# umutdundar99/progressive-stable-diffusion

Measured on AMD Instinct MI355X. Metric: images/sec at 512x512, 50 DDIM steps, bs/GPU=4, higher is better.
Workload: dtype f16; 1 GPU; 512x512, 50 DDIM steps, bs=4/GPU, delta-steer lambda=3.0, routing gates on, conditioning prep + VAE decode included; global_batch=4, parallelism=batch-shard x1 + 1 all-gather of uint8 frames

## Files before the change

### progressive-stable-diffusion_amd/csrc/conv_halo.hip

```cpp
#include <cstdlib>
#include <type_traits>

#include "dadd_common.h"
#include "igemm_args.h"
#include "igemm_epilogue.h"

#ifndef DADD_IGEMM_EXP
#define DADD_IGEMM_EXP 0
#endif
#if DADD_IGEMM_EXP == 3
#define DADD_STAMP(var) const unsigned long long var = __builtin_amdgcn_s_memtime()
#define DADD_ACC(dst, a, b) dst += (b) - (a)
#else
#define DADD_STAMP(var)
#define DADD_ACC(dst, a, b)
#endif

namespace {

constexpr int BM = 128, BK = 64, BN = 160;
constexpr int WN = BN / 2, J = WN / 16, NBJ = BN / 32;
constexpr int B_BYTES = BN * BK * 2;
constexpr int W_RING = 4 * B_BYTES;
constexpr int HALO_MAX_PIX = 272;
// ... 250 lines not shown
        __builtin_amdgcn_sched_barrier(0);
      }
      ++gi;
      __builtin_amdgcn_sched_barrier(0);
    };
    for (int c = c0; c < c1; ++c) {
      tap2(std::integral_constant<int, 0>{});
      tap2(std::integral_constant<int, 1>{});
      tap2(std::integral_constant<int, 2>{});
      tap2(std::integral_constant<int, 3>{});
      tap2(std::integral_constant<int, 4>{});
      tap2(std::integral_constant<int, 5>{});
      tap2(std::integral_constant<int, 6>{});
      tap2(std::integral_constant<int, 7>{});
      tap2(std::integral_constant<int, 8>{});
      const char* sw = hb;
      hb = hbo;
      hbo = sw;
    }
    __builtin_amdgcn_s_barrier();
    f4* park = reinterpret_cast<f4*>(smem + wave * (J * 4 * 64 * 16));
    if (wave_all >= 4) {
#pragma unroll
      for (int j = 0; j < J; ++j)
#pragma unroll
        for (int i = 0; i < 4; ++i) park[(j * 4 + i) * 64 + lane] = acc[j][i];
    }
    __builtin_amdgcn_s_barrier();
    if (wave_all >= 4) return;
#pragma unroll
    for (int j = 0; j < J; ++j)
#pragma unroll
      for (int i = 0; i < 4; ++i) acc[j][i] += park[(j * 4 + i) * 64 + lane];
    igemm_epilogue<J, 4, 64, WN>(p, acc, m0, n0, wm, wn, lane, z, smem, nullptr, nullptr, smem + GN_OFF);
    return;
  }
  if constexpr (GNIN) {
    const int cg = Cin >> 5;
    const int g = wave * 8 + (lane >> 3), sub = lane & 7;
    const bool second = p.C2 > 0 && g * cg >= p.C1;
    const float* wsp = second ? p.gni_ws2 : p.gni_ws;
    const int nch = second ? p.gni_nchunk2 : p.gni_nchunk;
    const int wsrc = (second ? p.C2 : p.C1) >> 5;
    const int r = p.C2 > 0 ? cg / wsrc : 1;
    const int g0 = p.C2 > 0 ? ((second ? g * cg - p.C1 : g * cg) / wsrc) : g;
    double a = 0.0, q = 0.0;
    for (int j = 0; j < r; ++j)
      for (int k = sub; k < nch; k += 32) {
        dadd_f2 v[4];
#pragma unroll
        for (int u = 0; u < 4; ++u) {
          const int kk = min(k + 8 * u, nch - 1);
          v[u] = *reinterpret_cast<const dadd_f2*>(wsp + (((size_t)b * nch + kk) * 32 + g0 + j) * 2);
        }
#pragma unroll
        for (int u = 0; u < 4; ++u) {
          if (k + 8 * u < nch) {
            a += (double)v[u][0];
            q += (double)v[u][1];
          }
        }
      }
#pragma unroll
    for (int o = 4; o > 0; o >>= 1) {
      a += __shfl_xor(a, o, 64);
      q += __shfl_xor(q, o, 64);
    }
// ... 112 lines not shown
```

### progressive-stable-diffusion_amd/csrc/igemm.hip

```cpp
#include "dadd_common.h"
#include "igemm_args.h"
#include <cstdlib>
#include <string>
#include "igemm_epilogue.h"

namespace {

constexpr int BM = 128;
constexpr int BK = 64;

__device__ __forceinline__ int lds_off(int row, int chunk) {
  return (row * 8 + (chunk ^ ((row >> 1) & 7))) * 8;
}

template <int BM, int BN, bool DEEP>
__global__ __launch_bounds__(256, 2) void igemm_kernel(const IgemmArgs p) {
  constexpr int WM = BM / 2;
  constexpr int MI = WM / 16;
  constexpr int WN = BN / 2;
  constexpr int J = WN / 16;
  constexpr int NA = BM * 8 / 256;
  constexpr int NB = BN * 8 / 256;
  extern __shared__ __attribute__((aligned(16))) char smem[];
  half_t* As = reinterpret_cast<half_t*>(smem);
  half_t* Bs = As + 2 * BM * BK;

  const int t = threadIdx.x, lane = t & 63, wave = t >> 6;
  const int wm = wave >> 1, wn = wave & 1;
  const int tile_id = xcd_remap(blockIdx.x, gridDim.x);
  int nt, mt;
  tile_decode_fast(p, tile_id, mt, nt);
  const int m0 = mt * BM, n0 = nt * BN;
  const int z = blockIdx.y;
  const int kt0 = z * p.kps;
  const int kt1 = min(p.nkt, kt0 + p.kps);
  const int Cin = p.C1 + p.C2;
  const int q = t & 7;
  const int r0 = t >> 3;
  const int Hv = p.ups ? 2 * p.Hi : p.Hi;
  const int Wv = p.ups ? 2 * p.Wi : p.Wi;
  const int HoWo = p.Ho * p.Wo;

  int a_pix[NA], a_y[NA], a_x[NA];
#pragma unroll
  for (int i = 0; i < NA; ++i) {
    const int m = m0 + r0 + 32 * i;
    const bool ok = m < p.M;
    const int mm = ok ? m : 0;
    int b, oy, ox;
    row_decode(p, mm, HoWo, b, oy, ox);
    a_pix[i] = b * p.Hi * p.Wi;
    a_y[i] = ok ? oy * p.stride - p.pad : -100000;
    a_x[i] = ox * p.stride - p.pad;
// ... 83 lines not shown
      const bool more = kt + 1 < kt1;
      if (more) gload(kt + 1, ra, rb);
      compute(cur);
      if (more) lstore(cur ^ 1, ra, rb);
      __syncthreads();
    }
  } else {
    h8 raA[NA], rbA[NB], raB[NA], rbB[NB];
    if (kt0 < kt1) {
      gload(kt0, raA, rbA);
      if (kt0 + 1 < kt1) gload(kt0 + 1, raB, rbB);
      lstore(0, raA, rbA);
    }
    __syncthreads();
    int kt = kt0;
    while (kt < kt1) {
      if (kt + 2 < kt1) gload(kt + 2, raA, rbA);
      compute(0);
      if (kt + 1 < kt1) lstore(1, raB, rbB);
      __syncthreads();
      if (++kt >= kt1) break;
      if (kt + 2 < kt1) gload(kt + 2, raB, rbB);
      compute(1);
      if (kt + 1 < kt1) lstore(0, raA, rbA);
      __syncthreads();
      ++kt;
    }
  }

  if (ln_stage) {
    asm volatile("s_waitcnt vmcnt(0)" ::: "memory");
    __syncthreads();
  }
  igemm_epilogue<J, MI, WM, WN>(p, acc, m0, n0, wm, wn, lane, z, smem, nullptr, nullptr, ln_scr, ln_sts ? ln_scr + LN_LDS_STATS : nullptr,
                                ln_stage ? ln_scr : nullptr);
}

__global__ __launch_bounds__(256) void splitk_finish_kernel(const IgemmArgs p, int nsplit) {
  const int n4 = p.N >> 2;
  const size_t total = (size_t)p.M * n4;
  const int HoWo = p.Ho * p.Wo;
  for (size_t idx = (size_t)blockIdx.x * blockDim.x + threadIdx.x; idx < total;
       idx += (size_t)gridDim.x * blockDim.x) {
    const int m = (int)(idx / n4);
    const int n = (int)(idx - (size_t)m * n4) * 4;
    f4 v = {0.f, 0.f, 0.f, 0.f};
    const float* slab = p.partial + (size_t)m * p.N + n;
    const size_t sstride = (size_t)p.M * p.N;
    int s = 0;
    for (; s + 4 <= nsplit; s += 4) {
      const f4 t0 = *reinterpret_cast<const f4*>(slab + (size_t)s * sstride);
      const f4 t1 = *reinterpret_cast<const f4*>(slab + (size_t)(s + 1) * sstride);
      const f4 t2 = *reinterpret_cast<const f4*>(slab + (size_t)(s + 2) * sstride);
      const f4 t3 = *reinterpret_cast<const f4*>(slab + (size_t)(s + 3) * sstride);
      v += t0;
      v += t1;
      v += t2;
      v += t3;
    }
    for (; s < nsplit; ++s) v += *reinterpret_cast<const f4*>(slab + (size_t)s * sstride);
    if (p.flags & DADD_EPI_BIAS) v += *reinterpret_cast<const f4*>(p.bias + n);
    if (p.flags & DADD_EPI_ROWVEC)
      v += *reinterpret_cast<const f4*>(p.rowvec + (size_t)(m / HoWo) * p.ld_rowvec + n);
    if (p.flags & DADD_EPI_RESIDUAL) {
      const h4 rv = *reinterpret_cast<const h4*>(p.residual + (size_t)m * p.ldr + n);
#pragma unroll
      for (int r = 0; r < 4; ++r) v[r] += (float)rv[r];
// ... 483 lines not shown
```

### progressive-stable-diffusion_amd/csrc/igemm_dma.hip

```cpp
#include "dadd_common.h"
#include "igemm_args.h"
#include <cstdlib>
#include "igemm_epilogue.h"

namespace {

constexpr int BK = 64;

typedef __attribute__((address_space(3))) void* lptr_t;
constexpr unsigned OOB = 0x80000000u;

__device__ __forceinline__ int lds_off(int row, int chunk) {
  return (row * 8 + (chunk ^ ((row >> 1) & 7))) * 8;
}

template <int N>
__device__ __forceinline__ void wait_vmcnt() {
  asm volatile("s_waitcnt vmcnt(%0)" ::"n"(N) : "memory");
}

template <int BM, int BN, bool UPS, bool PERS, int LNK>
__global__ __launch_bounds__(512, (BM + BN) <= 128 ? 4 : 2) void igemm_dma_kernel(const IgemmArgs p) {
#if defined(__HIP_DEVICE_COMPILE__)
  constexpr bool WS = true;
  constexpr bool LNF = LNK == 1;
  constexpr int WM = BM / 2, MI = WM / 16;
  constexpr int WN = BN / 2;
  constexpr int J = WN / 16;
  constexpr int NA = BM / 32;
  constexpr int NBJ = BN / 32;
  constexpr int LPT = NA + NBJ;
  constexpr int A_BYTES = BM * BK * 2, B_BYTES = BN * BK * 2, STAGE = A_BYTES + B_BYTES;
  extern __shared__ __attribute__((aligned(1024))) char smem[];

  const int t = threadIdx.x, lane = t & 63;
  const int wave_all = __builtin_amdgcn_readfirstlane(t >> 6);
  const bool loader = WS && wave_all >= 4;
  const int wave = WS ? (wave_all & 3) : wave_all;
  const int wm = wave >> 1, wn = wave & 1;
  int tile_first, tile_count;
  if constexpr (PERS) {
    const int total = p.mtiles * p.ntiles, nwg = gridDim.x;
    const int l = xcd_remap(blockIdx.x, nwg);
    const int q = total / nwg, r = total - q * nwg;
    tile_first = l * q + min(l, r);
    tile_count = q + (l < r ? 1 : 0);
  } else {
    tile_first = xcd_remap(blockIdx.x, gridDim.x);
    tile_count = 1;
  }
  const int z = PERS ? 0 : blockIdx.y;
  const int kt0 = PERS ? 0 : z * p.kps;
  const int kt1 = PERS ? p.nkt : min(p.nkt, kt0 + p.kps);
  const int nk = kt1 - kt0;
  const int Cin = p.C1 + p.C2;
  const int Hv = UPS ? 2 * p.Hi : p.Hi;
  const int Wv = UPS ? 2 * p.Wi : p.Wi;
  const int HoWo = p.Ho * p.Wo;
  const int lrow = lane >> 3, lch = lane & 7;

  const int shift1 = UPS ? 0 : (p.pad * p.Wi + p.pad) * p.C1;
// ... 249 lines not shown
        acc[jj][ii] = DADD_MFMA_16X16X32(wb0[jj], xa0[ii], acc[jj][ii], 0, 0, 0);
        if constexpr (LNF) {
#pragma unroll
          for (int t2 = 0; t2 < LPER; ++t2)
            if (k * LPER + t2 < LQ) ln_acc_pair(xa0[(k * LPER + t2) / 4], (k * LPER + t2) % 4, ls1[(k * LPER + t2) / 4], ls2[(k * LPER + t2) / 4]);
        }
        if (k == 0) wb1[0] = *reinterpret_cast<const h8*>(cb1);
        else if (k <= MI) xa1[k - 1] = *reinterpret_cast<const h8*>(ca + (k - 1) * 2048);
        else if (k < MI + J) wb1[k - MI] = *reinterpret_cast<const h8*>(cb1 + (k - MI) * 2048);
        __builtin_amdgcn_sched_barrier(0);
      }
#pragma unroll
      for (int k = 0; k < MI * J; ++k) {
        const int jj = k / MI, ii = k % MI;
        acc[jj][ii] = DADD_MFMA_16X16X32(wb1[jj], xa1[ii], acc[jj][ii], 0, 0, 0);
        if constexpr (LNF) {
#pragma unroll
          for (int t2 = 0; t2 < LPER; ++t2)
            if (k * LPER + t2 < LQ) ln_acc_pair(xa1[(k * LPER + t2) / 4], (k * LPER + t2) % 4, ls1[(k * LPER + t2) / 4], ls2[(k * LPER + t2) / 4]);
        }
        if (k == 0) wb0[0] = *reinterpret_cast<const h8*>(nb);
        else if (k <= MI) xa0[k - 1] = *reinterpret_cast<const h8*>(na + (k - 1) * 2048);
        else if (k < MI + J) wb0[k - MI] = *reinterpret_cast<const h8*>(nb + (k - MI) * 2048);
        __builtin_amdgcn_sched_barrier(0);
      }
      comp_off = next_off;
      __builtin_amdgcn_sched_barrier(0);
    }
    dadd_pf_drain(pf_sink);
    int nt, mt;
    tile_decode_fast(p, tile_first + tl, mt, nt);
    if constexpr (LNF) {
      ln_finish<MI>(ls1, ls2, p.K, p.ln_eps);
      igemm_epilogue<J, MI, WM, WN>(p, acc, mt * BM, nt * BN, wm, wn, lane, z, smem, ls1, ls2);
    } else {
      igemm_epilogue<J, MI, WM, WN>(p, acc, mt * BM, nt * BN, wm, wn, lane, z, smem, nullptr, nullptr, smem + 4 * STAGE,
                                    ln_sts ? ln_scr + LN_LDS_STATS : nullptr, ln_stage ? ln_scr : nullptr);
    }
  }
#endif
}

constexpr int smem_bytes(int bm, int bn) {
  return 4 * (bm + bn) * BK * 2 + (bm == 128 ? LN_LDS_BYTES : 4096);
}

#define DMA_ROW(BM, BN, UPS, PERS, LNK)                                                                                \
  {DADD_KNAME("igemm_dma_kernel") "<" #BM ", " #BN ", " #UPS ", " #PERS ", " #LNK ">", igemm_dma_kernel<BM, BN, UPS, PERS, LNK>, \
   512, smem_bytes(BM, BN), {BM, BN, UPS, PERS, LNK}}
#define DMA_ROWS2(BM, BN, PERS) DMA_ROW(BM, BN, false, PERS, 0), DMA_ROW(BM, BN, false, PERS, 1)
#define DMA_ROWS3(BM, BN, PERS) DMA_ROWS2(BM, BN, PERS), DMA_ROW(BM, BN, false, PERS, 2)
const IgemmKernel DMA_KERNELS[] = {
    DMA_ROWS3(128, 128, true),  DMA_ROWS3(128, 160, true),
    DMA_ROWS3(128, 128, false), DMA_ROWS3(128, 160, false),
    DMA_ROW(128, 128, true, false, 0), DMA_ROW(128, 160, true, false, 0),
    DMA_ROWS2(64, 64, false), DMA_ROWS2(64, 128, false), DMA_ROWS2(64, 160, false),
};
#undef DMA_ROWS3
#undef DMA_ROWS2
#undef DMA_ROW

}

int dadd_init_igemm_dma() { return dadd_set_max_lds(DMA_KERNELS); }

const IgemmKernel* dadd_igemm_dma_row(int tile_m, int tile_n, bool ups, bool persistent, int lnk) {
  return dadd_find_row(DMA_KERNELS, tile_m, tile_n, ups, persistent, lnk);
}
```

### progressive-stable-diffusion_amd/csrc/igemm_epilogue.h

```cpp
#pragma once
#include "igemm_args.h"
#include "ln_lds.h"

__device__ __forceinline__ float dadd_row16_sum(float v) {
  v += __builtin_bit_cast(float, __builtin_amdgcn_update_dpp(0, __builtin_bit_cast(int, v), 0xB1, 0xF, 0xF, true));
  v += __builtin_bit_cast(float, __builtin_amdgcn_update_dpp(0, __builtin_bit_cast(int, v), 0x4E, 0xF, 0xF, true));
  v += __builtin_bit_cast(float, __builtin_amdgcn_update_dpp(0, __builtin_bit_cast(int, v), 0x141, 0xF, 0xF, true));
  v += __builtin_bit_cast(float, __builtin_amdgcn_update_dpp(0, __builtin_bit_cast(int, v), 0x140, 0xF, 0xF, true));
  return v;
}

template <int J, int MI, int WM, int WN>
__device__ __forceinline__ void igemm_epilogue(const IgemmArgs& p, f4 (&acc)[J][MI], int m0, int n0,
                                               int wm, int wn, int lane, int z, char* smem,
                                               const float* ln_mu = nullptr, const float* ln_rs = nullptr,
                                               char* gn_scratch = nullptr, const char* ln_lds = nullptr,
                                               const char* ln_cb = nullptr) {
  const int g = lane >> 4, mc = lane & 15;
  const int HoWo = p.Ho * p.Wo;
  if (p.splitk > 1) {
#pragma unroll
    for (int i = 0; i < MI; ++i) {
      const int m = m0 + wm * WM + i * 16 + mc;
      if (m >= p.M) continue;
#pragma unroll
      for (int j = 0; j < J; ++j) {
        const int n = n0 + wn * WN + j * 16 + g * 4;
        if (n < p.N) *reinterpret_cast<f4*>(p.partial + ((size_t)z * p.M + m) * p.N + n) = acc[j][i];
      }
    }
    if (p.counters == nullptr) return;
    asm volatile("s_waitcnt vmcnt(0)" ::: "memory");
    __syncthreads();
    volatile int* flag = reinterpret_cast<volatile int*>(smem);
    if (threadIdx.x == 0) {
      __builtin_amdgcn_fence(__ATOMIC_RELEASE, "agent");
      asm volatile("s_waitcnt vmcnt(0)" ::: "memory");
      int* ticket = p.counters + blockIdx.x;
      const int prev = __hip_atomic_fetch_add(ticket, 1, __ATOMIC_RELAXED, __HIP_MEMORY_SCOPE_AGENT);
      const int last = (prev == p.splitk - 1) ? 1 : 0;
      if (last) {
        __builtin_amdgcn_fence(__ATOMIC_ACQUIRE, "agent");
        asm volatile("s_waitcnt vmcnt(0)" ::: "memory");
        __hip_atomic_store(ticket, 0, __ATOMIC_RELAXED, __HIP_MEMORY_SCOPE_AGENT);
      }
      *flag = last;
    }
    __syncthreads();
    if (*flag == 0) return;
#pragma unroll
    for (int i = 0; i < MI; ++i) {
      const int m = m0 + wm * WM + i * 16 + mc;
#pragma unroll
      for (int j = 0; j < J; ++j) {
        const int n = n0 + wn * WN + j * 16 + g * 4;
        f4 v = {0.f, 0.f, 0.f, 0.f};
        if (m < p.M && n < p.N)
          for (int s = 0; s < p.splitk; ++s)
            v += *reinterpret_cast<const f4*>(p.partial + ((size_t)s * p.M + m) * p.N + n);
        acc[j][i] = v;
      }
    }
  }
  if (p.flags & DADD_EPI_GNSTAT) {
    float* scratch = reinterpret_cast<float*>(gn_scratch) + (wm * 2 + wn) * 256;
    const int mrow0 = m0 + wm * WM;
    const int bsmp = row_sample(p, mrow0, HoWo);
#pragma unroll
    for (int j = 0; j < J; ++j) {
      const int n = n0 + wn * WN + j * 16 + g * 4;
      f4 bias4 = {0.f, 0.f, 0.f, 0.f};
      if (p.flags & DADD_EPI_BIAS) bias4 = *reinterpret_cast<const f4*>(p.bias + n);
      if (p.flags & DADD_EPI_ROWVEC) bias4 += *reinterpret_cast<const f4*>(p.rowvec + (size_t)bsmp * p.ld_rowvec + n);
      float cs[4] = {0.f, 0.f, 0.f, 0.f}, cq[4] = {0.f, 0.f, 0.f, 0.f};
#pragma unroll
      for (int i = 0; i < MI; ++i) {
        const int m = mrow0 + i * 16 + mc;
        f4 v = acc[j][i] + bias4;
        if (p.flags & DADD_EPI_RESIDUAL) {
          const h4 rv = *reinterpret_cast<const h4*>(p.residual + (size_t)m * p.ldr + n);
#pragma unroll
          for (int r = 0; r < 4; ++r) v[r] += (float)rv[r];
        }
        h4 o;
#pragma unroll
        for (int r = 0; r < 4; ++r) {
          o[r] = (half_t)v[r];
          const float f = (float)o[r];
          cs[r] += f;
          cq[r] = fmaf(f, f, cq[r]);
        }
        *reinterpret_cast<h4*>(p.out + (size_t)m * p.ldo + n) = o;
      }
#pragma unroll
      for (int r = 0; r < 4; ++r) {
        cs[r] = dadd_row16_sum(cs[r]);
        cq[r] = dadd_row16_sum(cq[r]);
      }
      if (mc == 0) {
#pragma unroll
        for (int r = 0; r < 4; ++r) {
          scratch[(j * 16 + g * 4 + r) * 2] = cs[r];
          scratch[(j * 16 + g * 4 + r) * 2 + 1] = cq[r];
        }
      }
    }
    __builtin_amdgcn_fence(__ATOMIC_RELEASE, "wavefront");
    __builtin_amdgcn_wave_barrier();
    __builtin_amdgcn_fence(__ATOMIC_ACQUIRE, "wavefront");
    const int ngrp = WN / p.gn_cg;
    if (lane < ngrp) {
      float a = 0.f, q = 0.f;
      for (int c = 0; c < p.gn_cg; ++c) {
        a += scratch[(lane * p.gn_cg + c) * 2];
        q += scratch[(lane * p.gn_cg + c) * 2 + 1];
      }
// ... 24 lines not shown
      mrow[i] = min(m0 + wm * WM + i * 16 + mc, p.M - 1);
    }
    if (ln_lds != nullptr) {
      for (int pp = 0; pp < p.ln_parts_in; ++pp)
#pragma unroll
        for (int i = 0; i < MI; ++i) {
          const dadd_f2 v = *reinterpret_cast<const dadd_f2*>(ln_lds + pp * 1024 + (wm * WM + i * 16 + mc) * 8);
          sa[i] += v[0];
          sq[i] += v[1];
        }
    } else
    for (int pp = 0; pp < p.ln_parts_in; pp += 4) {
      dadd_f2 v[4][MI];
#pragma unroll
      for (int u = 0; u < 4; ++u)
#pragma unroll
        for (int i = 0; i < MI; ++i)
          v[u][i] = st[(size_t)min(pp + u, p.ln_parts_in - 1) * p.M + mrow[i]];
#pragma unroll
      for (int u = 0; u < 4; ++u) {
        const float keep = (pp + u < p.ln_parts_in) ? 1.f : 0.f;
#pragma unroll
        for (int i = 0; i < MI; ++i) {
          sa[i] = fmaf(keep, v[u][i][0], sa[i]);
          sq[i] = fmaf(keep, v[u][i][1], sq[i]);
        }
      }
    }
    const float inv = __builtin_amdgcn_rcpf((float)p.K);
#pragma unroll
    for (int i = 0; i < MI; ++i) {
      const float mu = sa[i] * inv;
      lmu[i] = mu;
      lrs[i] = rsqrtf(fmaxf(sq[i] * inv - mu * mu, 0.f) + p.ln_eps);
    }
    fold = true;
  } else {
#pragma unroll
    for (int i = 0; i < MI; ++i) lmu[i] = 0.f, lrs[i] = 1.f;
  }
  if (fold && ln_cb != nullptr) {
#pragma unroll
    for (int i = 0; i < MI; ++i) {
      const int m = m0 + wm * WM + i * 16 + mc;
      if (m >= p.M) continue;
      if (p.flags & DADD_EPI_GEGLU) {
        if constexpr (J == 4) {
#pragma unroll
          for (int j = 0; j < 2; ++j) {
            const int ch = wn * WN + j * 16 + g * 4, cg2 = ch + 32;
            if (n0 + cg2 >= p.N) continue;
            f4 hv = lrs[i] * (acc[j][i] - lmu[i] * *reinterpret_cast<const f4*>(ln_cb + ch * 4));
            f4 gv = lrs[i] * (acc[j + 2][i] - lmu[i] * *reinterpret_cast<const f4*>(ln_cb + cg2 * 4));
            if (p.flags & DADD_EPI_BIAS) {
              hv += *reinterpret_cast<const f4*>(ln_cb + 1024 + ch * 4);
              gv += *reinterpret_cast<const f4*>(ln_cb + 1024 + cg2 * 4);
            }
            const int no = (n0 >> 1) + wn * 32 + j * 16 + g * 4;
            const dadd_f2 g01 = dadd_gelu2(dadd_f2{gv[0], gv[1]}), g23 = dadd_gelu2(dadd_f2{gv[2], gv[3]});
            const h4 o = {(half_t)(hv[0] * g01[0]), (half_t)(hv[1] * g01[1]), (half_t)(hv[2] * g23[0]),
                          (half_t)(hv[3] * g23[1])};
            *reinterpret_cast<h4*>(p.out + (size_t)m * p.ldo + no) = o;
          }
        }
        continue;
      }
#pragma unroll
      for (int j = 0; j < J; ++j) {
        const int c = wn * WN + j * 16 + g * 4, n = n0 + c;
        if (n >= p.N) continue;
        f4 v = lrs[i] * (acc[j][i] - lmu[i] * *reinterpret_cast<const f4*>(ln_cb + c * 4));
        if (p.flags & DADD_EPI_BIAS) v += *reinterpret_cast<const f4*>(ln_cb + 1024 + c * 4);
        if (p.flags & DADD_EPI_ROWVEC) v += *reinterpret_cast<const f4*>(p.rowvec + (size_t)row_sample(p, m, HoWo) * p.ld_rowvec + n);
        if (p.flags & DADD_EPI_ACT_MASK) {
          if (p.flags & DADD_EPI_QUICKGELU) {
#pragma unroll
            for (int r = 0; r < 4; ++r) v[r] = v[r] / (1.0f + __expf(-1.702f * v[r]));
          } else if (p.flags & DADD_EPI_GELU) {
#pragma unroll
            for (int r = 0; r < 4; ++r) v[r] = dadd_gelu(v[r]);
          } else {
#pragma unroll
            for (int r = 0; r < 4; ++r) v[r] = 1.0f / (1.0f + __expf(-v[r]));
          }
        }
        if (p.flags & DADD_EPI_RESIDUAL) {
          const h4 rv = *reinterpret_cast<const h4*>(p.residual + (size_t)m * p.ldr + n);
#pragma unroll
          for (int r = 0; r < 4; ++r) v[r] += (float)rv[r];
        }
        const h4 o = {(half_t)v[0], (half_t)v[1], (half_t)v[2], (half_t)v[3]};
        *reinterpret_cast<h4*>(p.out + (size_t)m * p.ldo + n) = o;
      }
    }
    return;
  }
  if (fold) {
    if (p.flags & DADD_EPI_GEGLU) {
      if constexpr (J == 4) {
#pragma unroll
        for (int j = 0; j < 2; ++j) {
          const int nh = n0 + wn * WN + j * 16 + g * 4;
          const int ng = nh + 32;
          if (ng >= p.N) continue;
          const f4 c1h = *reinterpret_cast<const f4*>(p.ln_c1 + nh), c1g = *reinterpret_cast<const f4*>(p.ln_c1 + ng);
          f4 bh = {0.f, 0.f, 0.f, 0.f}, bg = {0.f, 0.f, 0.f, 0.f};
          if (p.flags & DADD_EPI_BIAS) {
            bh = *reinterpret_cast<const f4*>(p.bias + nh);
            bg = *reinterpret_cast<const f4*>(p.bias + ng);
          }
          const int no = (n0 >> 1) + wn * 32 + j * 16 + g * 4;
#pragma unroll
          for (int i = 0; i < MI; ++i) {
            const int m = m0 + wm * WM + i * 16 + mc;
            if (m >= p.M) continue;
            const f4 hv = lrs[i] * (acc[j][i] - lmu[i] * c1h) + bh;
            const f4 gv = lrs[i] * (acc[j + 2][i] - lmu[i] * c1g) + bg;
            const dadd_f2 g01 = dadd_gelu2(dadd_f2{gv[0], gv[1]}), g23 = dadd_gelu2(dadd_f2{gv[2], gv[3]});
            const h4 o = {(half_t)(hv[0] * g01[0]), (half_t)(hv[1] * g01[1]), (half_t)(hv[2] * g23[0]),
                          (half_t)(hv[3] * g23[1])};
            *reinterpret_cast<h4*>(p.out + (size_t)m * p.ldo + no) = o;
          }
        }
      }
      return;
    }
#pragma unroll
    for (int j = 0; j < J; ++j) {
      const int n = n0 + wn * WN + j * 16 + g * 4;
      if (n >= p.N) continue;
      const f4 c4 = *reinterpret_cast<const f4*>(p.ln_c1 + n);
      f4 b4 = {0.f, 0.f, 0.f, 0.f};
      if (p.flags & DADD_EPI_BIAS) b4 = *reinterpret_cast<const f4*>(p.bias + n);
#pragma unroll
      for (int i = 0; i < MI; ++i) {
        const int m = m0 + wm * WM + i * 16 + mc;
        if (m >= p.M) continue;
        f4 v = lrs[i] * (acc[j][i] - lmu[i] * c4) + b4;
        if (p.flags & DADD_EPI_ROWVEC) v += *reinterpret_cast<const f4*>(p.rowvec + (size_t)row_sample(p, m, HoWo) * p.ld_rowvec + n);
        if (p.flags & DADD_EPI_ACT_MASK) {
          if (p.flags & DADD_EPI_QUICKGELU) {
#pragma unroll
            for (int r = 0; r < 4; ++r) v[r] = v[r] / (1.0f + __expf(-1.702f * v[r]));
          } else if (p.flags & DADD_EPI_GELU) {
#pragma unroll
            for (int r = 0; r < 4; ++r) v[r] = dadd_gelu(v[r]);
          } else {
#pragma unroll
            for (int r = 0; r < 4; ++r) v[r] = 1.0f / (1.0f + __expf(-v[r]));
          }
        }
        if (p.flags & DADD_EPI_RESIDUAL) {
          const h4 rv = *reinterpret_cast<const h4*>(p.residual + (size_t)m * p.ldr + n);
#pragma unroll
          for (int r = 0; r < 4; ++r) v[r] += (float)rv[r];
        }
        const h4 o = {(half_t)v[0], (half_t)v[1], (half_t)v[2], (half_t)v[3]};
        *reinterpret_cast<h4*>(p.out + (size_t)m * p.ldo + n) = o;
      }
    }
    return;
  }
  const bool lnstat = (p.flags & DADD_EPI_LNSTAT) != 0 && n0 + wn * WN < p.N;
#pragma unroll
  for (int i = 0; i < MI; ++i) {
    const int m = m0 + wm * WM + i * 16 + mc;
    if (m >= p.M) continue;
    const int b = (p.flags & DADD_EPI_ROWVEC) ? row_sample(p, m, HoWo) : 0;
    float rs1 = 0.f, rs2 = 0.f;
    if (p.flags & DADD_EPI_GEGLU) {
      if constexpr (J == 4) {
#pragma unroll
        for (int j = 0; j < 2; ++j) {
          const int nh = n0 + wn * WN + j * 16 + g * 4;
          const int ng = nh + 32;
          if (ng >= p.N) continue;
          f4 hv = acc[j][i], gv = acc[j + 2][i];
          if (p.flags & DADD_EPI_BIAS) {
            hv += *reinterpret_cast<const f4*>(p.bias + nh);
            gv += *reinterpret_cast<const f4*>(p.bias + ng);
          }
          const int no = (n0 >> 1) + wn * 32 + j * 16 + g * 4;
          const dadd_f2 g01 = dadd_gelu2(dadd_f2{gv[0], gv[1]}), g23 = dadd_gelu2(dadd_f2{gv[2], gv[3]});
          const h4 o = {(half_t)(hv[0] * g01[0]), (half_t)(hv[1] * g01[1]), (half_t)(hv[2] * g23[0]),
                        (half_t)(hv[3] * g23[1])};
          *reinterpret_cast<h4*>(p.out + (size_t)m * p.ldo + no) = o;
        }
      }
      continue;
    }
#pragma unroll
    for (int j = 0; j < J; ++j) {
      const int n = n0 + wn * WN + j * 16 + g * 4;
      if (n >= p.N) continue;
      f4 v = acc[j][i];
      if (p.flags & DADD_EPI_BIAS) v += *reinterpret_cast<const f4*>(p.bias + n);
      if (p.flags & DADD_EPI_ROWVEC) v += *reinterpret_cast<const f4*>(p.rowvec + (size_t)b * p.ld_rowvec + n);
      if (p.flags & DADD_EPI_ACT_MASK) {
        if (p.flags & DADD_EPI_QUICKGELU) {
#pragma unroll
          for (int r = 0; r < 4; ++r) v[r] = v[r] / (1.0f + __expf(-1.702f * v[r]));
        } else if (p.flags & DADD_EPI_GELU) {
#pragma unroll
          for (int r = 0; r < 4; ++r) v[r] = dadd_gelu(v[r]);
        } else {
#pragma unroll
          for (int r = 0; r < 4; ++r) v[r] = 1.0f / (1.0f + __expf(-v[r]));
        }
      }
      if (p.flags & DADD_EPI_RESIDUAL) {
        const h4 rv = *reinterpret_cast<const h4*>(p.residual + (size_t)m * p.ldr + n);
#pragma unroll
        for (int r = 0; r < 4; ++r) v[r] += (float)rv[r];
      }
      h4 o;
#pragma unroll
      for (int r = 0; r < 4; ++r) {
        o[r] = (half_t)v[r];
        const float f = (float)o[r];
        rs1 += f;
        rs2 = fmaf(f, f, rs2);
      }
      *reinterpret_cast<h4*>(p.out + (size_t)m * p.ldo + n) = o;
    }
    if (lnstat) {
      rs1 = dadd_sum_x16x32(rs1);
      rs2 = dadd_sum_x16x32(rs2);
      if (g == 0) {
        const int part = (n0 + wn * WN) / WN;
        reinterpret_cast<dadd_f2*>(p.ln_stats_out)[(size_t)part * p.M + m] = dadd_f2{rs1, rs2};
      }
    }
  }
}
```

Before: 11.34 images/sec.

## Restructure GEMM epilogue to batch operand loads by tile, row or column

Rewrites the shared GEMM/conv epilogue so bias, rowvec, LN-fold constants and residual loads are hoisted into register arrays. They are issued in batches: the whole tile up front, per row, or per column, with the mode picked at compile time for each kernel variant. Indices are clamped so loads need no guards, and additions use selects. The aim is more memory-level parallelism and less latency exposed in the store-heavy epilogue. The cost is higher register pressure, which could lower occupancy, plus some slight changes to rounding and FMA contraction.

```diff
diff --git a/progressive-stable-diffusion_amd/csrc/conv_halo.hip b/progressive-stable-diffusion_amd/csrc/conv_halo.hip
--- a/progressive-stable-diffusion_amd/csrc/conv_halo.hip
+++ b/progressive-stable-diffusion_amd/csrc/conv_halo.hip
@@ -306,7 +306,7 @@
     for (int j = 0; j < J; ++j)
 #pragma unroll
       for (int i = 0; i < 4; ++i) acc[j][i] += park[(j * 4 + i) * 64 + lane];
-    igemm_epilogue<J, 4, 64, WN>(p, acc, m0, n0, wm, wn, lane, z, smem, nullptr, nullptr, smem + GN_OFF);
+    igemm_epilogue<J, 4, 64, WN, EPI_COLS>(p, acc, m0, n0, wm, wn, lane, z, smem, nullptr, nullptr, smem + GN_OFF);
     return;
   }
   if constexpr (GNIN) {
diff --git a/progressive-stable-diffusion_amd/csrc/igemm.hip b/progressive-stable-diffusion_amd/csrc/igemm.hip
--- a/progressive-stable-diffusion_amd/csrc/igemm.hip
+++ b/progressive-stable-diffusion_amd/csrc/igemm.hip
@@ -19,6 +19,7 @@
   constexpr int MI = WM / 16;
   constexpr int WN = BN / 2;
   constexpr int J = WN / 16;
+  constexpr int EPI = (DEEP && BN == 128) ? EPI_COLS : EPI_TILE;
   constexpr int NA = BM * 8 / 256;
   constexpr int NB = BN * 8 / 256;
   extern __shared__ __attribute__((aligned(16))) char smem[];
@@ -168,7 +169,8 @@
     asm volatile("s_waitcnt vmcnt(0)" ::: "memory");
     __syncthreads();
   }
-  igemm_epilogue<J, MI, WM, WN>(p, acc, m0, n0, wm, wn, lane, z, smem, nullptr, nullptr, ln_scr, ln_sts ? ln_scr + LN_LDS_STATS : nullptr,
+  const int lane_e = __builtin_amdgcn_mbcnt_hi(~0u, __builtin_amdgcn_mbcnt_lo(~0u, 0u));
+  igemm_epilogue<J, MI, WM, WN, EPI>(p, acc, m0, n0, wm, wn, lane_e, z, smem, nullptr, nullptr, ln_scr, ln_sts ? ln_scr + LN_LDS_STATS : nullptr,
                                 ln_stage ? ln_scr : nullptr);
 }
 
diff --git a/progressive-stable-diffusion_amd/csrc/igemm_dma.hip b/progressive-stable-diffusion_amd/csrc/igemm_dma.hip
--- a/progressive-stable-diffusion_amd/csrc/igemm_dma.hip
+++ b/progressive-stable-diffusion_amd/csrc/igemm_dma.hip
@@ -27,6 +27,7 @@
   constexpr int WM = BM / 2, MI = WM / 16;
   constexpr int WN = BN / 2;
   constexpr int J = WN / 16;
+  constexpr int EPI = !PERS ? EPI_TILE : (BN == 160 && LNK == 2) ? EPI_COLS : EPI_ROWS;
   constexpr int NA = BM / 32;
   constexpr int NBJ = BN / 32;
   constexpr int LPT = NA + NBJ;
@@ -342,9 +343,9 @@
     tile_decode_fast(p, tile_first + tl, mt, nt);
     if constexpr (LNF) {
       ln_finish<MI>(ls1, ls2, p.K, p.ln_eps);
-      igemm_epilogue<J, MI, WM, WN>(p, acc, mt * BM, nt * BN, wm, wn, lane, z, smem, ls1, ls2);
+      igemm_epilogue<J, MI, WM, WN, EPI>(p, acc, mt * BM, nt * BN, wm, wn, lane, z, smem, ls1, ls2);
     } else {
-      igemm_epilogue<J, MI, WM, WN>(p, acc, mt * BM, nt * BN, wm, wn, lane, z, smem, nullptr, nullptr, smem + 4 * STAGE,
+      igemm_epilogue<J, MI, WM, WN, EPI>(p, acc, mt * BM, nt * BN, wm, wn, lane, z, smem, nullptr, nullptr, smem + 4 * STAGE,
                                     ln_sts ? ln_scr + LN_LDS_STATS : nullptr, ln_stage ? ln_scr : nullptr);
     }
   }
diff --git a/progressive-stable-diffusion_amd/csrc/igemm_epilogue.h b/progressive-stable-diffusion_amd/csrc/igemm_epilogue.h
--- a/progressive-stable-diffusion_amd/csrc/igemm_epilogue.h
+++ b/progressive-stable-diffusion_amd/csrc/igemm_epilogue.h
@@ -1,6 +1,153 @@
 #pragma once
 #include "igemm_args.h"
 #include "ln_lds.h"
+#include <type_traits>
+
+__device__ __forceinline__ f4 epi_add_if(bool on, const f4& v, const f4& b) {
+#pragma clang fp contract(off)
+  const f4 s = v + b;
+  return on ? s : v;
+}
+__device__ __forceinline__ f4 epi_add_if(bool on, const f4& v, const h4& b) {
+#pragma clang fp contract(off)
+  const f4 s = {v[0] + (float)b[0], v[1] + (float)b[1], v[2] + (float)b[2], v[3] + (float)b[3]};
+  return on ? s : v;
+}
+__device__ __forceinline__ void epi_activate(int flags, f4& v) {
+  if (flags & DADD_EPI_QUICKGELU) {
+#pragma unroll
+    for (int r = 0; r < 4; ++r) v[r] = v[r] / (1.0f + __expf(-1.702f * v[r]));
+  } else if (flags & DADD_EPI_GELU) {
+#pragma unroll
+    for (int r = 0; r < 4; ++r) v[r] = dadd_gelu(v[r]);
+  } else {
+#pragma unroll
+    for (int r = 0; r < 4; ++r) v[r] = 1.0f / (1.0f + __expf(-v[r]));
+  }
+}
+
+constexpr bool epi_ln_var_fused(int J, int MI, int i) { return MI == 2 || (J == 4 && i >= 2); }
+__device__ __forceinline__ float epi_ln_var(bool fused, float ex2, float mu) {
+#pragma clang fp contract(off)
+  const float mu2 = mu * mu;
+  return fused ? fmaf(-mu, mu, ex2) : ex2 - mu2;
+}
+
+enum { EPI_TILE = 0, EPI_ROWS = 1, EPI_COLS = 2 };
+
+template <int J, int MI, int MODE>
+struct EpiOperands {
+  int mcl[MI], ncl[J];
+  f4 b4[J], c4[J], r4[J];
+  f4 rq[MI];
+  h4 res[J][MI];
+  bool has_bias, has_rv, has_res, has_c1, rv_one;
+  int b0;
+
+  __device__ __forceinline__ void init(const IgemmArgs& p, int mw, int nw, int mc, int g, int HoWo, bool with_bias,
+                                       bool with_c1) {
+    has_bias = with_bias && (p.flags & DADD_EPI_BIAS) != 0;
+    has_c1 = with_c1;
+    has_rv = (p.flags & DADD_EPI_ROWVEC) != 0;
+    has_res = (p.flags & DADD_EPI_RESIDUAL) != 0;
+#pragma unroll
+    for (int i = 0; i < MI; ++i) {
+      mcl[i] = min(mw + i * 16 + mc, p.M - 1);
+      rq[i] = f4{0.f, 0.f, 0.f, 0.f};
+    }
+#pragma unroll
+    for (int j = 0; j < J; ++j) {
+      ncl[j] = min(nw + j * 16 + g * 4, p.N - 4);
+      b4[j] = c4[j] = r4[j] = f4{0.f, 0.f, 0.f, 0.f};
+#pragma unroll
+      for (int i = 0; i < MI; ++i) res[j][i] = h4{};
+    }
+    b0 = 0;
+    rv_one = false;
+    if (has_rv) {
+      b0 = row_sample(p, min(mw, p.M - 1), HoWo);
+      rv_one = b0 == row_sample(p, min(mw + MI * 16 - 1, p.M - 1), HoWo);
+    }
+  }
+  __device__ __forceinline__ void load_col(const IgemmArgs& p, int j) {
+    if (has_c1) c4[j] = *reinterpret_cast<const f4*>(p.ln_c1 + ncl[j]);
+    if (has_bias) b4[j] = *reinterpret_cast<const f4*>(p.bias + ncl[j]);
+    if (rv_one) r4[j] = *reinterpret_cast<const f4*>(p.rowvec + (size_t)b0 * p.ld_rowvec + ncl[j]);
+  }
+  __device__ __forceinline__ void load_res(const IgemmArgs& p, int i, int j) {
+    res[j][i] = *reinterpret_cast<const h4*>(p.residual + (size_t)mcl[i] * p.ldr + ncl[j]);
+  }
+  __device__ __forceinline__ void before(const IgemmArgs& p) {
+    if constexpr (MODE != EPI_COLS) {
+      if (has_c1) {
+#pragma unroll
+        for (int j = 0; j < J; ++j) c4[j] = *reinterpret_cast<const f4*>(p.ln_c1 + ncl[j]);
+      }
+      if (has_bias) {
+#pragma unroll
+        for (int j = 0; j < J; ++j) b4[j] = *reinterpret_cast<const f4*>(p.bias + ncl[j]);
+      }
+      if (rv_one) {
+#pragma unroll
+        for (int j = 0; j < J; ++j) r4[j] = *reinterpret_cast<const f4*>(p.rowvec + (size_t)b0 * p.ld_rowvec + ncl[j]);
+      }
+    }
+    if constexpr (MODE == EPI_TILE) {
+      if (has_res) {
+#pragma unroll
+        for (int i = 0; i < MI; ++i)
+#pragma unroll
+          for (int j = 0; j < J; ++j) load_res(p, i, j);
+      }
+    }
+  }
+  __device__ __forceinline__ void batch(const IgemmArgs& p, int o, int HoWo) {
+    if constexpr (MODE == EPI_COLS) {
+      load_col(p, o);
+      if (has_rv && !rv_one) {
+#pragma unroll
+        for (int i = 0; i < MI; ++i)
+          rq[i] = *reinterpret_cast<const f4*>(p.rowvec + (size_t)row_sample(p, mcl[i], HoWo) * p.ld_rowvec + ncl[o]);
+      }
+      if (has_res) {
+#pragma unroll
+        for (int i = 0; i < MI; ++i) load_res(p, i, o);
+      }
+    } else {
+      if (has_rv && !rv_one) {
+        const float* row = p.rowvec + (size_t)row_sample(p, mcl[o], HoWo) * p.ld_rowvec;
+#pragma unroll
+        for (int j = 0; j < J; ++j) r4[j] = *reinterpret_cast<const f4*>(row + ncl[j]);
+      }
+      if constexpr (MODE == EPI_ROWS) {
+        if (has_res) {
+#pragma unroll
+          for (int j = 0; j < J; ++j) load_res(p, o, j);
+        }
+      }
+    }
+  }
+  __device__ __forceinline__ f4 rowvec(int i, int j) const {
+    if constexpr (MODE == EPI_COLS) return rv_one ? r4[j] : rq[i];
+    return r4[j];
+  }
+};
+
+template <int J, int MI, int MODE, class B, class E, class R>
+__device__ __forceinline__ void epi_for_each(B&& batch, E&& elem, R&& row_done) {
+  constexpr bool COLS = MODE == EPI_COLS;
+#pragma unroll
+  for (int o = 0; o < (COLS ? J : MI); ++o) {
+    batch(o);
+#pragma unroll
+    for (int q = 0; q < (COLS ? MI : J); ++q) elem(COLS ? q : o, COLS ? o : q);
+    if constexpr (!COLS) row_done(o);
+  }
+  if constexpr (COLS) {
+#pragma unroll
+    for (int i = 0; i < MI; ++i) row_done(i);
+  }
+}
 
 __device__ __forceinline__ float dadd_row16_sum(float v) {
   v += __builtin_bit_cast(float, __builtin_amdgcn_update_dpp(0, __builtin_bit_cast(int, v), 0xB1, 0xF, 0xF, true));
@@ -10,7 +157,60 @@
   return v;
 }
 
-template <int J, int MI, int WM, int WN>
+enum { EPI_PLAIN = 0, EPI_FOLD_GLOBAL = 1, EPI_FOLD_LDS = 2 };
+template <int J, int MI, int WM, int WN, int MODE, int FOLD>
+__device__ __forceinline__ void epi_tile(const IgemmArgs& p, f4 (&acc)[J][MI], int m0, int n0, int wm, int wn, int g, int mc,
+                                         int HoWo, const float (&lmu)[MI], const float (&lrs)[MI], const char* ln_cb) {
+  const bool lnstat = FOLD == EPI_PLAIN && (p.flags & DADD_EPI_LNSTAT) != 0 && n0 + wn * WN < p.N;
+  EpiOperands<J, MI, MODE> ops;
+  ops.init(p, m0 + wm * WM, n0 + wn * WN, mc, g, HoWo, FOLD != EPI_FOLD_LDS, FOLD == EPI_FOLD_GLOBAL);
+  ops.before(p);
+  float rs1[MI], rs2[MI];
+#pragma unroll
+  for (int i = 0; i < MI; ++i) rs1[i] = rs2[i] = 0.f;
+  epi_for_each<J, MI, MODE>(
+      [&](int o) __attribute__((always_inline)) { ops.batch(p, o, HoWo); },
+      [&](int i, int j) __attribute__((always_inline)) {
+        const int m = m0 + wm * WM + i * 16 + mc;
+        const int c = wn * WN + j * 16 + g * 4, n = n0 + c;
+        if (m >= p.M || n >= p.N) return;
+        f4 v;
+        if constexpr (FOLD == EPI_FOLD_LDS) {
+          v = lrs[i] * (acc[j][i] - lmu[i] * *reinterpret_cast<const f4*>(ln_cb + c * 4));
+          if (p.flags & DADD_EPI_BIAS) v += *reinterpret_cast<const f4*>(ln_cb + 1024 + c * 4);
+        } else if constexpr (FOLD == EPI_FOLD_GLOBAL) {
+          v = lrs[i] * (acc[j][i] - lmu[i] * ops.c4[j]) + ops.b4[j];
+        } else {
+          v = epi_add_if(ops.has_bias, acc[j][i], ops.b4[j]);
+        }
+        v = epi_add_if(ops.has_rv, v, ops.rowvec(i, j));
+        if (p.flags & DADD_EPI_ACT_MASK) epi_activate(p.flags, v);
+        v = epi_add_if(ops.has_res, v, ops.res[j][i]);
+        h4 o;
+#pragma unroll
+        for (int r = 0; r < 4; ++r) {
+          o[r] = (half_t)v[r];
+          if constexpr (FOLD == EPI_PLAIN) {
+            const float f = (float)o[r];
+            rs1[i] += f;
+            rs2[i] = fmaf(f, f, rs2[i]);
+          }
+        }
+        *reinterpret_cast<h4*>(p.out + (size_t)m * p.ldo + n) = o;
+      },
+      [&](int i) __attribute__((always_inline)) {
+        const int m = m0 + wm * WM + i * 16 + mc;
+        if (lnstat && m < p.M) {
+          const float t1 = dadd_sum_x16x32(rs1[i]), t2 = dadd_sum_x16x32(rs2[i]);
+          if (g == 0) {
+            const int part = (n0 + wn * WN) / WN;
+            reinterpret_cast<dadd_f2*>(p.ln_stats_out)[(size_t)part * p.M + m] = dadd_f2{t1, t2};
+          }
+        }
+      });
+}
+
+template <int J, int MI, int WM, int WN, int MODE = EPI_TILE>
 __device__ __forceinline__ void igemm_epilogue(const IgemmArgs& p, f4 (&acc)[J][MI], int m0, int n0,
                                                int wm, int wn, int lane, int z, char* smem,
                                                const float* ln_mu = nullptr, const float* ln_rs = nullptr,
@@ -66,22 +266,51 @@
     float* scratch = reinterpret_cast<float*>(gn_scratch) + (wm * 2 + wn) * 256;
     const int mrow0 = m0 + wm * WM;
     const int bsmp = row_sample(p, mrow0, HoWo);
+    const bool has_bias = (p.flags & DADD_EPI_BIAS) != 0, has_rv = (p.flags & DADD_EPI_ROWVEC) != 0;
+    const bool has_res = (p.flags & DADD_EPI_RESIDUAL) != 0;
+    f4 b4[J], r4[J];
+    h4 res[J][MI];
+#pragma unroll
+    for (int j = 0; j < J; ++j) {
+      b4[j] = r4[j] = f4{0.f, 0.f, 0.f, 0.f};
+#pragma unroll
+      for (int i = 0; i < MI; ++i) res[j][i] = h4{};
+    }
+    auto load_blocks = [&](int ja, int jb) __attribute__((always_inline)) {
+      const int nw = n0 + wn * WN + g * 4;
+      if (has_bias) {
+#pragma unroll
+        for (int j = 0; j < J; ++j)
+          if (j >= ja && j < jb) b4[j] = *reinterpret_cast<const f4*>(p.bias + nw + j * 16);
+      }
+      if (has_rv) {
+#pragma unroll
+        for (int j = 0; j < J; ++j)
+          if (j >= ja && j < jb) r4[j] = *reinterpret_cast<const f4*>(p.rowvec + (size_t)bsmp * p.ld_rowvec + nw + j * 16);
+      }
+      if (has_res) {
+#pragma unroll
+        for (int i = 0; i < MI; ++i)
+#pragma unroll
+          for (int j = 0; j < J; ++j)
+            if (j >= ja && j < jb)
+              res[j][i] = *reinterpret_cast<const h4*>(p.residual + (size_t)(mrow0 + i * 16 + mc) * p.ldr + nw + j * 16);
+      }
+    };
+    if constexpr (MODE == EPI_TILE) load_blocks(0, J);
 #pragma unroll
     for (int j = 0; j < J; ++j) {
       const int n = n0 + wn * WN + j * 16 + g * 4;
+      if constexpr (MODE != EPI_TILE) load_blocks(j, j + 1);
       f4 bias4 = {0.f, 0.f, 0.f, 0.f};
-      if (p.flags & DADD_EPI_BIAS) bias4 = *reinterpret_cast<const f4*>(p.bias + n);
-      if (p.flags & DADD_EPI_ROWVEC) bias4 += *reinterpret_cast<const f4*>(p.rowvec + (size_t)bsmp * p.ld_rowvec + n);
+      if (has_bias) bias4 = b4[j];
+      bias4 = epi_add_if(has_rv, bias4, r4[j]);
       float cs[4] = {0.f, 0.f, 0.f, 0.f}, cq[4] = {0.f, 0.f, 0.f, 0.f};
 #pragma unroll
       for (int i = 0; i < MI; ++i) {
         const int m = mrow0 + i * 16 + mc;
         f4 v = acc[j][i] + bias4;
-        if (p.flags & DADD_EPI_RESIDUAL) {
-          const h4 rv = *reinterpret_cast<const h4*>(p.residual + (size_t)m * p.ldr + n);
-#pragma unroll
-          for (int r = 0; r < 4; ++r) v[r] += (float)rv[r];
-        }
+        v = epi_add_if(has_res, v, res[j][i]);
         h4 o;
 #pragma unroll
         for (int r = 0; r < 4; ++r) {
@@ -172,153 +401,29 @@
     for (int i = 0; i < MI; ++i) {
       const float mu = sa[i] * inv;
       lmu[i] = mu;
-      lrs[i] = rsqrtf(fmaxf(sq[i] * inv - mu * mu, 0.f) + p.ln_eps);
+      lrs[i] = rsqrtf(fmaxf(epi_ln_var(epi_ln_var_fused(J, MI, i), sq[i] * inv, mu), 0.f) + p.ln_eps);
     }
     fold = true;
   } else {
 #pragma unroll
     for (int i = 0; i < MI; ++i) lmu[i] = 0.f, lrs[i] = 1.f;
   }
-  if (fold && ln_cb != nullptr) {
+  const bool lds_fold = fold && ln_cb != nullptr;
+  if (lds_fold && (p.flags & DADD_EPI_GEGLU)) {
 #pragma unroll
     for (int i = 0; i < MI; ++i) {
       const int m = m0 + wm * WM + i * 16 + mc;
       if (m >= p.M) continue;
-      if (p.flags & DADD_EPI_GEGLU) {
-        if constexpr (J == 4) {
-#pragma unroll
-          for (int j = 0; j < 2; ++j) {
-            const int ch = wn * WN + j * 16 + g * 4, cg2 = ch + 32;
-            if (n0 + cg2 >= p.N) continue;
-            f4 hv = lrs[i] * (acc[j][i] - lmu[i] * *reinterpret_cast<const f4*>(ln_cb + ch * 4));
-            f4 gv = lrs[i] * (acc[j + 2][i] - lmu[i] * *reinterpret_cast<const f4*>(ln_cb + cg2 * 4));
-            if (p.flags & DADD_EPI_BIAS) {
-              hv += *reinterpret_cast<const f4*>(ln_cb + 1024 + ch * 4);
-              gv += *reinterpret_cast<const f4*>(ln_cb + 1024 + cg2 * 4);
-            }
-            const int no = (n0 >> 1) + wn * 32 + j * 16 + g * 4;
-            const dadd_f2 g01 = dadd_gelu2(dadd_f2{gv[0], gv[1]}), g23 = dadd_gelu2(dadd_f2{gv[2], gv[3]});
-            const h4 o = {(half_t)(hv[0] * g01[0]), (half_t)(hv[1] * g01[1]), (half_t)(hv[2] * g23[0]),
-                          (half_t)(hv[3] * g23[1])};
-            *reinterpret_cast<h4*>(p.out + (size_t)m * p.ldo + no) = o;
-          }
-        }
-        continue;
-      }
-#pragma unroll
-      for (int j = 0; j < J; ++j) {
-        const int c = wn * WN + j * 16 + g * 4, n = n0 + c;
-        if (n >= p.N) continue;
-        f4 v = lrs[i] * (acc[j][i] - lmu[i] * *reinterpret_cast<const f4*>(ln_cb + c * 4));
-        if (p.flags & DADD_EPI_BIAS) v += *reinterpret_cast<const f4*>(ln_cb + 1024 + c * 4);
-        if (p.flags & DADD_EPI_ROWVEC) v += *reinterpret_cast<const f4*>(p.rowvec + (size_t)row_sample(p, m, HoWo) * p.ld_rowvec + n);
-        if (p.flags & DADD_EPI_ACT_MASK) {
-          if (p.flags & DADD_EPI_QUICKGELU) {
-#pragma unroll
-            for (int r = 0; r < 4; ++r) v[r] = v[r] / (1.0f + __expf(-1.702f * v[r]));
-          } else if (p.flags & DADD_EPI_GELU) {
-#pragma unroll
-            for (int r = 0; r < 4; ++r) v[r] = dadd_gelu(v[r]);
-          } else {
-#pragma unroll
-            for (int r = 0; r < 4; ++r) v[r] = 1.0f / (1.0f + __expf(-v[r]));
-          }
-        }
-        if (p.flags & DADD_EPI_RESIDUAL) {
-          const h4 rv = *reinterpret_cast<const h4*>(p.residual + (size_t)m * p.ldr + n);
-#pragma unroll
-          for (int r = 0; r < 4; ++r) v[r] += (float)rv[r];
-        }
-        const h4 o = {(half_t)v[0], (half_t)v[1], (half_t)v[2], (half_t)v[3]};
-        *reinterpret_cast<h4*>(p.out + (size_t)m * p.ldo + n) = o;
-      }
-    }
-    return;
-  }
-  if (fold) {
-    if (p.flags & DADD_EPI_GEGLU) {
       if constexpr (J == 4) {
 #pragma unroll
         for (int j = 0; j < 2; ++j) {
-          const int nh = n0 + wn * WN + j * 16 + g * 4;
-          const int ng = nh + 32;
-          if (ng >= p.N) continue;
-          const f4 c1h = *reinterpret_cast<const f4*>(p.ln_c1 + nh), c1g = *reinterpret_cast<const f4*>(p.ln_c1 + ng);
-          f4 bh = {0.f, 0.f, 0.f, 0.f}, bg = {0.f, 0.f, 0.f, 0.f};
+          const int ch = wn * WN + j * 16 + g * 4, cg2 = ch + 32;
+          if (n0 + cg2 >= p.N) continue;
+          f4 hv = lrs[i] * (acc[j][i] - lmu[i] * *reinterpret_cast<const f4*>(ln_cb + ch * 4));
+          f4 gv = lrs[i] * (acc[j + 2][i] - lmu[i] * *reinterpret_cast<const f4*>(ln_cb + cg2 * 4));
           if (p.flags & DADD_EPI_BIAS) {
-            bh = *reinterpret_cast<const f4*>(p.bias + nh);
-            bg = *reinterpret_cast<const f4*>(p.bias + ng);
-          }
-          const int no = (n0 >> 1) + wn * 32 + j * 16 + g * 4;
-#pragma unroll
-          for (int i = 0; i < MI; ++i) {
-            const int m = m0 + wm * WM + i * 16 + mc;
-            if (m >= p.M) continue;
-            const f4 hv = lrs[i] * (acc[j][i] - lmu[i] * c1h) + bh;
-            const f4 gv = lrs[i] * (acc[j + 2][i] - lmu[i] * c1g) + bg;
-            const dadd_f2 g01 = dadd_gelu2(dadd_f2{gv[0], gv[1]}), g23 = dadd_gelu2(dadd_f2{gv[2], gv[3]});
-            const h4 o = {(half_t)(hv[0] * g01[0]), (half_t)(hv[1] * g01[1]), (half_t)(hv[2] * g23[0]),
-                          (half_t)(hv[3] * g23[1])};
-            *reinterpret_cast<h4*>(p.out + (size_t)m * p.ldo + no) = o;
-          }
-        }
-      }
-      return;
-    }
-#pragma unroll
-    for (int j = 0; j < J; ++j) {
-      const int n = n0 + wn * WN + j * 16 + g * 4;
-      if (n >= p.N) continue;
-      const f4 c4 = *reinterpret_cast<const f4*>(p.ln_c1 + n);
-      f4 b4 = {0.f, 0.f, 0.f, 0.f};
-      if (p.flags & DADD_EPI_BIAS) b4 = *reinterpret_cast<const f4*>(p.bias + n);
-#pragma unroll
-      for (int i = 0; i < MI; ++i) {
-        const int m = m0 + wm * WM + i * 16 + mc;
-        if (m >= p.M) continue;
-        f4 v = lrs[i] * (acc[j][i] - lmu[i] * c4) + b4;
-        if (p.flags & DADD_EPI_ROWVEC) v += *reinterpret_cast<const f4*>(p.rowvec + (size_t)row_sample(p, m, HoWo) * p.ld_rowvec + n);
-        if (p.flags & DADD_EPI_ACT_MASK) {
-          if (p.flags & DADD_EPI_QUICKGELU) {
-#pragma unroll
-            for (int r = 0; r < 4; ++r) v[r] = v[r] / (1.0f + __expf(-1.702f * v[r]));
-          } else if (p.flags & DADD_EPI_GELU) {
-#pragma unroll
-            for (int r = 0; r < 4; ++r) v[r] = dadd_gelu(v[r]);
-          } else {
-#pragma unroll
-            for (int r = 0; r < 4; ++r) v[r] = 1.0f / (1.0f + __expf(-v[r]));
-          }
-        }
-        if (p.flags & DADD_EPI_RESIDUAL) {
-          const h4 rv = *reinterpret_cast<const h4*>(p.residual + (size_t)m * p.ldr + n);
-#pragma unroll
-          for (int r = 0; r < 4; ++r) v[r] += (float)rv[r];
-        }
-        const h4 o = {(half_t)v[0], (half_t)v[1], (half_t)v[2], (half_t)v[3]};
-        *reinterpret_cast<h4*>(p.out + (size_t)m * p.ldo + n) = o;
-      }
-    }
-    return;
-  }
-  const bool lnstat = (p.flags & DADD_EPI_LNSTAT) != 0 && n0 + wn * WN < p.N;
-#pragma unroll
-  for (int i = 0; i < MI; ++i) {
-    const int m = m0 + wm * WM + i * 16 + mc;
-    if (m >= p.M) continue;
-    const int b = (p.flags & DADD_EPI_ROWVEC) ? row_sample(p, m, HoWo) : 0;
-    float rs1 = 0.f, rs2 = 0.f;
-    if (p.flags & DADD_EPI_GEGLU) {
-      if constexpr (J == 4) {
-#pragma unroll
-        for (int j = 0; j < 2; ++j) {
-          const int nh = n0 + wn * WN + j * 16 + g * 4;
-          const int ng = nh + 32;
-          if (ng >= p.N) continue;
-          f4 hv = acc[j][i], gv = acc[j + 2][i];
-          if (p.flags & DADD_EPI_BIAS) {
-            hv += *reinterpret_cast<const f4*>(p.bias + nh);
-            gv += *reinterpret_cast<const f4*>(p.bias + ng);
+            hv += *reinterpret_cast<const f4*>(ln_cb + 1024 + ch * 4);
+            gv += *reinterpret_cast<const f4*>(ln_cb + 1024 + cg2 * 4);
           }
           const int no = (n0 >> 1) + wn * 32 + j * 16 + g * 4;
           const dadd_f2 g01 = dadd_gelu2(dadd_f2{gv[0], gv[1]}), g23 = dadd_gelu2(dadd_f2{gv[2], gv[3]});
@@ -327,49 +432,62 @@
           *reinterpret_cast<h4*>(p.out + (size_t)m * p.ldo + no) = o;
         }
       }
-      continue;
-    }
-#pragma unroll
-    for (int j = 0; j < J; ++j) {
-      const int n = n0 + wn * WN + j * 16 + g * 4;
-      if (n >= p.N) continue;
-      f4 v = acc[j][i];
-      if (p.flags & DADD_EPI_BIAS) v += *reinterpret_cast<const f4*>(p.bias + n);
-      if (p.flags & DADD_EPI_ROWVEC) v += *reinterpret_cast<const f4*>(p.rowvec + (size_t)b * p.ld_rowvec + n);
-      if (p.flags & DADD_EPI_ACT_MASK) {
-        if (p.flags & DADD_EPI_QUICKGELU) {
-#pragma unroll
-          for (int r = 0; r < 4; ++r) v[r] = v[r] / (1.0f + __expf(-1.702f * v[r]));
-        } else if (p.flags & DADD_EPI_GELU) {
-#pragma unroll
-          for (int r = 0; r < 4; ++r) v[r] = dadd_gelu(v[r]);
-        } else {
-#pragma unroll
-          for (int r = 0; r < 4; ++r) v[r] = 1.0f / (1.0f + __expf(-v[r]));
-        }
-      }
-      if (p.flags & DADD_EPI_RESIDUAL) {
-        const h4 rv = *reinterpret_cast<const h4*>(p.residual + (size_t)m * p.ldr + n);
-#pragma unroll
-        for (int r = 0; r < 4; ++r) v[r] += (float)rv[r];
-      }
-      h4 o;
-#pragma unroll
-      for (int r = 0; r < 4; ++r) {
-        o[r] = (half_t)v[r];
-        const float f = (float)o[r];
-        rs1 += f;
-        rs2 = fmaf(f, f, rs2);
-      }
-      *reinterpret_cast<h4*>(p.out + (size_t)m * p.ldo + n) = o;
-    }
-    if (lnstat) {
-      rs1 = dadd_sum_x16x32(rs1);
-      rs2 = dadd_sum_x16x32(rs2);
-      if (g == 0) {
-        const int part = (n0 + wn * WN) / WN;
-        reinterpret_cast<dadd_f2*>(p.ln_stats_out)[(size_t)part * p.M + m] = dadd_f2{rs1, rs2};
-      }
-    }
-  }
-}
+    }
+    return;
+  }
+  if (p.flags & DADD_EPI_GEGLU) {
+    if constexpr (J == 4) {
+      const bool has_bias = (p.flags & DADD_EPI_BIAS) != 0;
+      auto geglu = [&](auto folded) __attribute__((always_inline)) {
+        constexpr bool FOLD = decltype(folded)::value, COLS = MODE == EPI_COLS;
+        f4 c1[J], b4[J];
+#pragma unroll
+        for (int j = 0; j < J; ++j) c1[j] = b4[j] = f4{0.f, 0.f, 0.f, 0.f};
+        auto load_pair = [&](int j) __attribute__((always_inline)) {
+          const int nh = min(n0 + wn * WN + j * 16 + g * 4, p.N - 4), ng = min(n0 + wn * WN + j * 16 + g * 4 + 32, p.N - 4);
+          if constexpr (FOLD) {
+            c1[j] = *reinterpret_cast<const f4*>(p.ln_c1 + nh);
+            c1[j + 2] = *reinterpret_cast<const f4*>(p.ln_c1 + ng);
+          }
+          if (has_bias) {
+            b4[j] = *reinterpret_cast<const f4*>(p.bias + nh);
+            b4[j + 2] = *reinterpret_cast<const f4*>(p.bias + ng);
+          }
+        };
+        if constexpr (!COLS) {
+          load_pair(0);
+          load_pair(1);
+        }
+#pragma unroll
+        for (int o = 0; o < (COLS ? 2 : MI); ++o) {
+          if constexpr (COLS) load_pair(o);
+#pragma unroll
+          for (int q = 0; q < (COLS ? MI : 2); ++q) {
+            const int i = COLS ? q : o, j = COLS ? o : q;
+            const int m = m0 + wm * WM + i * 16 + mc;
+            if (m >= p.M || n0 + wn * WN + j * 16 + g * 4 + 32 >= p.N) continue;
+            f4 hv, gv;
+            if constexpr (FOLD) {
+              hv = lrs[i] * (acc[j][i] - lmu[i] * c1[j]) + b4[j];
+              gv = lrs[i] * (acc[j + 2][i] - lmu[i] * c1[j + 2]) + b4[j + 2];
+            } else {
+              hv = epi_add_if(has_bias, acc[j][i], b4[j]);
+              gv = epi_add_if(has_bias, acc[j + 2][i], b4[j + 2]);
+            }
+            const int no = (n0 >> 1) + wn * 32 + j * 16 + g * 4;
+            const dadd_f2 g01 = dadd_gelu2(dadd_f2{gv[0], gv[1]}), g23 = dadd_gelu2(dadd_f2{gv[2], gv[3]});
+            const h4 o4 = {(half_t)(hv[0] * g01[0]), (half_t)(hv[1] * g01[1]), (half_t)(hv[2] * g23[0]),
+                           (half_t)(hv[3] * g23[1])};
+            *reinterpret_cast<h4*>(p.out + (size_t)m * p.ldo + no) = o4;
+          }
+        }
+      };
+      if (fold) geglu(std::true_type{});
+      else geglu(std::false_type{});
+    }
+    return;
+  }
+  if (lds_fold) epi_tile<J, MI, WM, WN, MODE, EPI_FOLD_LDS>(p, acc, m0, n0, wm, wn, g, mc, HoWo, lmu, lrs, ln_cb);
+  else if (fold) epi_tile<J, MI, WM, WN, MODE, EPI_FOLD_GLOBAL>(p, acc, m0, n0, wm, wn, g, mc, HoWo, lmu, lrs, ln_cb);
+  else epi_tile<J, MI, WM, WN, MODE, EPI_PLAIN>(p, acc, m0, n0, wm, wn, g, mc, HoWo, lmu, lrs, ln_cb);
+}
```

Result: faster. 11.47 images/sec (median of 6 runs) (+1.1%).
